# syzhang092218-source/dgppo

Measured on AMD Instinct MI355X. Metric: env-steps/sec whole node, LidarSpread n=8 4096 envs, 1/2/4/8 GPUs, higher is better.
Workload: dtype f32

## Files before the change

dgppo_amd/csrc/nn_dense.hip:

```cpp
#include "common.h"
#include "nn_gru.h"

using f32x4 = __attribute__((ext_vector_type(4))) float;
#ifdef DGPPO_STAMPS
__device__ unsigned long long g_dstamps[32];
#define DSTAMP(i) do { if (blockIdx.x == 0 && threadIdx.x == 0) g_dstamps[i] = __builtin_amdgcn_s_memtime(); } while (0)
extern "C" int32_t dgppo_debug_stamps_dense(unsigned long long* out) {
  return (int32_t)hipMemcpyFromSymbol(out, HIP_SYMBOL(g_dstamps), sizeof(unsigned long long) * 32);
}
#else
#define DSTAMP(i)
#endif

#define DENSE_ROWS 64

struct DenseArgs {
  const float* X; int ldx;
  const float* W; int ldw;
  const float* bias;
  float* Y; int ldy;
  int M, K, N;
  int act;
  int accumulate;
  int trans_w;
// ... 1015 lines not shown
  const float* dhn;
  float* dWi; int ldwi;
  float* dbi;
  float* dWh; int ldwh;
  float* dbhn;
  int M, rows_per_block;
  float* part;
  const float* dhs;
  const float* gates;
  float* dgi_out;
  GruH0Map hmap;
};

template <bool T1>
__global__ void __launch_bounds__(512) gru_bwd_w_kernel(GruBwdWArgs a) {
  extern __shared__ float sm[];
  const int tid = threadIdx.x, lane = tid & 63, wave = (tid >> 6) & 3, half = tid >> 8;
  const int li = lane & 15, lq = lane >> 4;
  const int m_begin = blockIdx.x * a.rows_per_block;
  const int m_end = min(a.M, m_begin + a.rows_per_block);
  f32x4 acc[12];
#pragma unroll
  for (int t = 0; t < 12; ++t) acc[t] = f32x4{0.f, 0.f, 0.f, 0.f};
  float4 pfa[2], pfy[T1 ? 6 : 4];
  float4 csum[T1 ? 4 : 1];
#pragma unroll
  for (int u = 0; u < (T1 ? 4 : 1); ++u) csum[u] = make_float4(0.f, 0.f, 0.f, 0.f);
  const int qa = tid & 31, ra = tid >> 5, qy = tid & 63, ry = tid >> 6;
  const int q1 = tid & 15, r1 = tid >> 4;
  auto hrow = [&](int row) -> const float* {
    if constexpr (T1) { if (a.hmap.n_inner.d > 0) return gru_h0_map_row(a.hprev, a.hmap, row); }
    return a.hprev + (size_t)row * a.ldh;
  };
  auto fetch = [&](int m0) {
#pragma unroll
    for (int u = 0; u < 2; ++u) {
      int row = m0 + u * 16 + ra;
      row = row < a.M ? row : a.M - 1;
      const float* src = qa < 16 ? a.x + (size_t)row * a.ldx + 4 * qa : hrow(row) + 4 * (qa - 16);
      pfa[u] = *reinterpret_cast<const float4*>(src);
    }
    if constexpr (T1) {
      int row = m0 + r1;
      row = row < a.M ? row : a.M - 1;
      pfy[0] = *reinterpret_cast<const float4*>(a.dhs + (size_t)row * 64 + 4 * q1);
      pfy[1] = *reinterpret_cast<const float4*>(hrow(row) + 4 * q1);
      const float* gs = a.gates + (size_t)row * 256 + 4 * q1;
#pragma unroll
      for (int g = 0; g < 4; ++g) pfy[2 + g] = *reinterpret_cast<const float4*>(gs + 64 * g);
    } else {
#pragma unroll
      for (int u = 0; u < 4; ++u) {
        int row = m0 + u * 8 + ry;
        row = row < a.M ? row : a.M - 1;
        const float* src = qy < 48 ? a.dgi + (size_t)row * 192 + 4 * qy : a.dhn + (size_t)row * 64 + 4 * (qy - 48);
        pfy[u] = *reinterpret_cast<const float4*>(src);
      }
    }
  };
  auto commit = [&](int m0, int b) {
    float* as = sm + b * GW_BUF;
    float* ys = as + BW_ROWS * GW_AL;
#pragma unroll
    for (int u = 0; u < 2; ++u) {
      const int r = u * 16 + ra;
      const float4 v = (m0 + r < m_end) ? pfa[u] : make_float4(0.f, 0.f, 0.f, 0.f);
      *reinterpret_cast<float4*>(as + r * GW_AL + 4 * qa) = v;
    }
    if constexpr (T1) {
      const bool in = m0 + r1 < m_end;
      const GruGateGrad g0 = gru_gate_grad(gru_zero_carry(pfy[0].x), pfy[1].x, pfy[2].x, pfy[3].x, pfy[4].x, pfy[5].x);
      const GruGateGrad g1 = gru_gate_grad(gru_zero_carry(pfy[0].y), pfy[1].y, pfy[2].y, pfy[3].y, pfy[4].y, pfy[5].y);
      const GruGateGrad g2 = gru_gate_grad(gru_zero_carry(pfy[0].z), pfy[1].z, pfy[2].z, pfy[3].z, pfy[4].z, pfy[5].z);
      const GruGateGrad g3 = gru_gate_grad(gru_zero_carry(pfy[0].w), pfy[1].w, pfy[2].w, pfy[3].w, pfy[4].w, pfy[5].w);
      float4 v[4] = {make_float4(g0.dar, g1.dar, g2.dar, g3.dar), make_float4(g0.daz, g1.daz, g2.daz, g3.daz),
                     make_float4(g0.dan, g1.dan, g2.dan, g3.dan), make_float4(g0.dhn, g1.dhn, g2.dhn, g3.dhn)};
      if (in) {
        float* o = a.dgi_out + (size_t)(m0 + r1) * 192 + 4 * q1;
#pragma unroll
        for (int g = 0; g < 3; ++g) *reinterpret_cast<float4*>(o + 64 * g) = v[g];
      }
#pragma unroll
      for (int g = 0; g < 4; ++g) {
        if (!in) v[g] = make_float4(0.f, 0.f, 0.f, 0.f);
        *reinterpret_cast<float4*>(ys + r1 * GW_YL + 64 * g + 4 * q1) = v[g];
        csum[g].x += v[g].x; csum[g].y += v[g].y; csum[g].z += v[g].z; csum[g].w += v[g].w;
      }
    } else {
#pragma unroll
      for (int u = 0; u < 4; ++u) {
        const int r = u * 8 + ry;
        const float4 v = (m0 + r < m_end) ? pfy[u] : make_float4(0.f, 0.f, 0.f, 0.f);
        *reinterpret_cast<float4*>(ys + r * GW_YL + 4 * qy) = v;
        csum[0].x += v.x; csum[0].y += v.y; csum[0].z += v.z; csum[0].w += v.w;
      }
    }
  };
  auto compute = [&](int b) {
    const float* as = sm + b * GW_BUF + lq * GW_AL + half * 64 + wave * 16 + li;
    const float* ys = sm + b * GW_BUF + BW_ROWS * GW_AL + lq * GW_YL + li;
    const float* yh = ys + (half ? 64 : 0);
#pragma unroll
    for (int s4 = 0; s4 < BW_ROWS / 4; ++s4) {
      float bv[12];
#pragma unroll
      for (int t = 0; t < 8; ++t) bv[t] = ys[s4 * 4 * GW_YL + t * 16];
#pragma unroll
      for (int t = 8; t < 12; ++t) bv[t] = yh[s4 * 4 * GW_YL + t * 16];
      const float av = as[s4 * 4 * GW_AL];
#pragma unroll
      for (int t = 0; t < 12; ++t) acc[t] = __builtin_amdgcn_mfma_f32_16x16x4f32(av, bv[t], acc[t], 0, 0, 0);
    }
  };
  fetch(m_begin);
  commit(m_begin, 0);
  __syncthreads();
  int cur = 0;
  for (int m0 = m_begin; m0 < m_end; m0 += BW_ROWS) {
    fetch(m0 + BW_ROWS);
    __builtin_amdgcn_sched_barrier(0);
    compute(cur);
    commit(m0 + BW_ROWS, cur ^ 1);
    asm volatile("s_waitcnt lgkmcnt(0)\n\ts_barrier" ::: "memory");
    cur ^= 1;
  }
  float* slab = a.part ? a.part + (size_t)blockIdx.x * GW_SLAB : nullptr;
  {
    float* out = half ? a.dWh : a.dWi;
    const int ldo = half ? a.ldwh : a.ldwi;
    float* sl = slab ? slab + (half ? GW_SLAB_WH : GW_SLAB_WI) : nullptr;
#pragma unroll
    for (int t = 0; t < 12; ++t) {
      const int col = t * 16 + li;
#pragma unroll
      for (int r = 0; r < 4; ++r) {
        const int krow = wave * 16 + lq * 4 + r;
// ... 193 lines not shown
```

dgppo_amd/csrc/nn_fused.hip:

```cpp
#include <type_traits>
#include "common.h"
#include "nn_ln.h"

using f32x4 = __attribute__((ext_vector_type(4))) float;
#define FZ_H 64
#define FZ_HL 66
#define FZ_RB 32
#define FZ_LDS_BARRIER() asm volatile("s_waitcnt lgkmcnt(0)\n\ts_barrier" ::: "memory")

__device__ inline float row16_sum(float v) {
  v += __int_as_float(__builtin_amdgcn_update_dpp(0, __float_as_int(v), 0xB1, 0xf, 0xf, false));
  v += __int_as_float(__builtin_amdgcn_update_dpp(0, __float_as_int(v), 0x4E, 0xf, 0xf, false));
  v += __int_as_float(__builtin_amdgcn_update_dpp(0, __float_as_int(v), 0x141, 0xf, 0xf, false));
  v += __int_as_float(__builtin_amdgcn_update_dpp(0, __float_as_int(v), 0x140, 0xf, 0xf, false));
  return v;
}

struct MlpGiArgs {
  const float* X; int ldx; int M;
  const float *W1, *b1, *g1, *be1, *W2, *b2, *g2, *be2, *Wi, *bi;
  float *p1, *y1, *st1, *p2, *y2, *st2;
  float* gi;
};

__global__ void __launch_bounds__(256) __attribute__((amdgpu_waves_per_eu(2, 8))) mlp_gi_fwd_kernel(MlpGiArgs a) {
// ... 1417 lines not shown
    else hipLaunchKernelGGL(gru1_head_fwd_rw_kernel<false>, dim3(grid_rw), dim3(64 * RW_WAVES), smem_rw, (hipStream_t)stream, a);
    DGPPO_LAUNCH_CHECK();
    return 0;
  }
  const size_t smem = sizeof(float) * 3 * FZ_RB * FZ_HL;
  const void* fn = two ? reinterpret_cast<const void*>(&gru1_head_fwd_kernel<true>)
                       : reinterpret_cast<const void*>(&gru1_head_fwd_kernel<false>);
  static thread_local int cap[2] = {0, 0};
  if (cap[two] == 0) {
    int per_cu = 0, dev = 0, cus = 256;
    if (hipOccupancyMaxActiveBlocksPerMultiprocessor(&per_cu, fn, 256, smem) != hipSuccess || per_cu < 1) per_cu = 1;
    if (hipGetDevice(&dev) != hipSuccess ||
        hipDeviceGetAttribute(&cus, hipDeviceAttributeMultiprocessorCount, dev) != hipSuccess || cus < 1) cus = 256;
    cap[two] = per_cu * cus;
  }
  const int tiles = (M + FZ_RB - 1) / FZ_RB;
  const int grid = tiles < cap[two] ? tiles : cap[two];
  if (two) hipLaunchKernelGGL(gru1_head_fwd_kernel<true>, dim3(grid), dim3(256), smem, (hipStream_t)stream, a);
  else hipLaunchKernelGGL(gru1_head_fwd_kernel<false>, dim3(grid), dim3(256), smem, (hipStream_t)stream, a);
  DGPPO_LAUNCH_CHECK();
  return 0;
}

#define HB_HL 68
#define HB_WAVES 8
#define HB_TILE (16 * HB_HL)
#define HB_BIG 1088
#define HB_SLAB_ONE HB_BIG
#define HB_SLAB_TWO (HB_BIG + FZ_H * FZ_H + FZ_H)
struct HeadBwdArgs {
  const float* feat; int ldf;
  const float* u;
  const float* dout; int n_out;
  const float *W1, *W2;
  float* dhs;
  float* dW1; int ldw1; float* db1;
  float* dW2; int ldw2; float* db2;
  float* part;
  int M;
};

template <bool TWO>
__global__ void __launch_bounds__(64 * HB_WAVES) head_bwd_kernel(HeadBwdArgs a) {
  extern __shared__ float sm[];
  const int tid = threadIdx.x, lane = tid & 63, w = tid >> 6, li = lane & 15, lq = lane >> 4;
  float* s_f = sm + w * 3 * HB_TILE;
// ... 244 lines not shown
```

dgppo_amd/engine.py:

```python
from __future__ import annotations

import dataclasses
from typing import Callable, Dict, Optional

import numpy as np
import os
import torch

from . import _native as N
from . import nets
from . import ops_algo as OA
from . import ops_env as OE
from . import ops_nn as K
from .utils import checkpoint as CK


@dataclasses.dataclass
class Hyper:
    gamma: float = 0.99
    gae_lambda: float = 0.95
    clip_eps: float = 0.25
    coef_ent: float = 1e-2
    max_grad_norm: float = 2.0
    lr_actor: float = 3e-4
# ... 404 lines not shown
                continue
            HC = self.HC
            hstar = self._final_carry(ro, e0, Eb)
            restore = False
            if not self.hp.use_rnn:
                h0 = None
            elif HC == H and self.carry_in_place:
                s0 = 0 if ro.stochastic else 1
                tm = ro._rnn_all
                if ro.stochastic:
                    tm[T + 1, e0:e0 + Eb].copy_(tm[T, e0:e0 + Eb])
                tm[s0 + T, e0:e0 + Eb].copy_(hstar.view(Eb, n, H))
                h0 = K.H0Map(tm[s0, e0:], tm.stride(1), tm.stride(0), T + 1, n, Eb, n_env_src=B - e0)
                restore = ro.stochastic
            elif HC == H:
                s0 = 0 if ro.stochastic else 1
                ro._rnn_em[e0:e0 + Eb, s0 + T].copy_(hstar.view(Eb, n, H))
                h0 = K.H0Blocks(ro._rnn_em[e0, s0], (T + 1) * n, (T + 2) * n * H, Eb)
            else:
                h0_all = self.arena.get("pre.h0all", Eb, T + 1, n, H)
                h0_all[:, :T].copy_(self._vh_carry(ro, e0, Eb))
                h0_all[:, T].copy_(hstar.view(Eb, n, HC)[..., :H])
                h0 = h0_all.view(-1, H)
            act = self.Vh.forward(feats, n_seq=Eb * (T + 1) * n, T=1, h0=h0, tag="pre", train=False)
            Vh_buf[e0:e0 + Eb].copy_(act["v"].view(Eb, T + 1, n, nh))
            if restore:
                ro._rnn_all[T, e0:e0 + Eb].copy_(ro._rnn_all[T + 1, e0:e0 + Eb])
        return Vl_buf, Vh_buf

    def require_landscape(self, what: str = "vh_landscape"):
        if self.algo != "dgppo":
            why = {"informarl_lagr": "its constraint-value net carries its own scan state, which needs a sequence pass first"}
            raise ValueError(f"{what}: algo '{self.algo}' is not supported: "
                             + why.get(self.algo, "it has no constraint-value network"))
        if self.cfg.is_vmas:
            raise ValueError(f"{what}: VMASReverseTransport is not supported")

    def vh_landscape(self, ro: RolloutData, env_index: int, agent_id: int, frame_ids, xs, ys,
                     events: Optional[list] = None) -> torch.Tensor:
        self.require_landscape()
        cfg, T = self.cfg, self.T
        n, nh, H = cfg.n_agents, self.n_cost, nets.HID
        ro.finalize()
        if not 0 <= int(env_index) < ro.B:
            raise ValueError(f"vh_landscape: env_index {env_index} outside [0, {ro.B})")
        if not 0 <= int(agent_id) < n:
            raise ValueError(f"vh_landscape: agent_id {agent_id} outside [0, {n})")
# ... 893 lines not shown
```

dgppo_amd/nets.py:

```python
from __future__ import annotations

import math
from typing import Dict, List, Optional, Tuple

import numpy as np
import torch

from . import _native as N
from . import ops_nn as K

H_HEADS = 3
MSG_DIM = 32
OUT_DIM = 64
HID = 64


def _ceil4(x):
    return (x + 3) // 4 * 4


class Layout:
    def __init__(self):
        self.entries: Dict[str, Tuple[int, Tuple[int, ...]]] = {}
        self.size = 0
# ... 192 lines not shown
    def pg(self, name):
        return self._cached("pg", self.prep_layout, self.prep_grads, name)

    def prepare(self):
        for l, (f, fp, d, kp) in enumerate(self.dims):
            q = lambda nm: self.p(f"gnn{l}.{nm}")
            K.gnn_prep(q("Wq"), q("bq"), q("Wk"), q("Wv"), q("bv"), q("We"), q("Wu"), self.pp(f"gnn{l}.Mcat"),
                       self.pp(f"gnn{l}.cvec"), self.pp(f"gnn{l}.Wout"), f, fp, d, H_HEADS, kp)

    def _xo_fusable(self, l: int) -> bool:
        if l != 0 or self.gnn_layers != 2:
            return False
        key = "_xo_ok"
        if not hasattr(self, key):
            f1, fp1, d1, kp1 = self.dims[1]
            setattr(self, key, self.dims[0][1] == 8 and self.dims[0][2] == 32 and fp1 == 32 and
                    K.attn_xo_supported(self.cfg, fp1, H_HEADS, kp1))
        return getattr(self, key)

    def zero_grads(self):
        self.grads.zero_()

    def forward(self, feats: GraphFeats, n_seq: int, T: int, h0: Optional[torch.Tensor], tag: str = "f",
                hs_out: Optional[torch.Tensor] = None, train: bool = True, qt0: Optional[torch.Tensor] = None):
        cfg, G, A = self.cfg, feats.G, self.arena
        n = cfg.n_agents
        R = G * n
        Ro = G * feats.n_other
        act = {"feats": feats, "G": G, "n_seq": n_seq, "T": T}
        Xa, Xo = feats.Xa, feats.Xo
        xo_fused = None
        for l, (f, fp, d, kp) in enumerate(self.dims):
            if l == 0 and qt0 is not None:
                assert tuple(qt0.shape) == (R, H_HEADS * fp), (tuple(qt0.shape), R, H_HEADS * fp)
                qt = qt0
            else:
                qt = A.get(f"{tag}.qt{l}", R, H_HEADS * fp)
                K.dense_fwd(Xa, self.pp(f"gnn{l}.Mcat"), self.pp(f"gnn{l}.cvec"), qt)
            zcat = A.get(f"{tag}.zcat{l}", R, kp)
            lean = l == 0 and self.lean_attn0 and feats.edges_from_rows
            attn = A.get(f"{tag}.attn{l}", R, cfg.fan_in, H_HEADS) if train and not lean else None
            if lean:
                K.attn_fwd_rows(cfg, fp, H_HEADS, kp, qt, Xa, Xo if Ro > 0 else None, feats.emask, zcat, None, G)
            elif xo_fused is not None:
                K.attn_fwd_xo(cfg, fp, H_HEADS, kp, qt, Xa, xo_fused[0], xo_fused[1], xo_fused[2], feats.efeat, feats.emask, zcat, attn, G)
            else:
                K.attn_fwd(cfg, fp, H_HEADS, kp, qt, Xa, Xo if Ro > 0 else None, feats.efeat, feats.emask, zcat, attn, G)
# ... 41 lines not shown
            saves = None
            if train:
                saves = tuple(A.get(f"{tag}.{nm}{i}", Rh, w) for i in (1, 2) for nm, w in (("p", HID), ("y", HID), ("st", 2)))
                for i in (1, 2):
                    act[f"p{i}"], act[f"y{i}"], act[f"st{i}"] = saves[3 * (i - 1):3 * i]
            K.mlp_gi_fwd(x, self.p("mlp.W1"), self.p("mlp.b1"), self.p("mlp.g1"), self.p("mlp.be1"), self.p("mlp.W2"),
                         self.p("mlp.b2"), self.p("mlp.g2"), self.p("mlp.be2"), self.p("gru.Wi"), self.p("gru.bi"), gi, saves)
        assert n_seq * T == Rh, (n_seq, T, Rh)
        L, CD = self.rnn_layers, self.carry_dim
        h0_blocks = isinstance(h0, K.H0Blocks)
        if h0_blocks:
            assert self.rnn == "gru" and L == 1 and T == 1 and not train and self.kind != "policy", \
                "a blocked h0 serves the one-cell GRU value nets' T = 1 inference pass"
        h0_map = isinstance(h0, K.H0Map)
        if h0_map:
            assert self.rnn == "gru" and L == 1 and T == 1 and self.kind != "policy" and h0.n_inner == n_inner, \
                "a mapped h0 serves the one-cell GRU value nets' T = 1 passes"
        elif h0 is not None and not h0_blocks:
            assert tuple(h0.shape) == (n_seq, CD), (tuple(h0.shape), n_seq, CD)
        if hs_out is not None:
            assert tuple(hs_out.shape) == (Rh, CD), (tuple(hs_out.shape), Rh, CD)
        act["gi"] = gi
        simple = (self.rnn == "gru" and L == 1)
        if simple:
            hs = hs_out if hs_out is not None else A.get(f"{tag}.hs", Rh, HID)
            hprev_is_h0 = train and T == 1 and h0 is not None and self.kind != "policy"
            hprev = A.get(f"{tag}.hprev", Rh, HID) if (train and not hprev_is_h0) else None
            gates = A.get(f"{tag}.gates", Rh, 4 * HID) if train else None
            feat = hs
            act["hs"], act["hprev"], act["gates"] = hs, hprev, gates
        fused_tail = (simple and T == 1 and self.kind == "policy")
        if simple and not fused_tail:
            if h0_blocks:
                K.gru_fwd_h0_blocks(gi, self.p("gru.Wh"), self.p("gru.bhn"), h0, hs, hprev, gates, n_seq, T, n_inner)
            elif h0_map:
                K.gru_fwd_h0_map(gi, self.p("gru.Wh"), self.p("gru.bhn"), h0, hs, hprev, gates, n_seq, T, n_inner)
            else:
                K.gru_fwd(gi, self.p("gru.Wh"), self.p("gru.bhn"), h0, hs, hprev, gates, n_seq, T, n_inner)
            if hprev_is_h0:
                act["hprev"] = act["h0"] = h0
        if self.rnn == "none":
            feat = act["y2"]
            if hs_out is not None:
                if h0 is not None and T == 1:
                    hs_out.copy_(h0)
                else:
                    hs_out.zero_()
        elif self.rnn == "lstm":
            x_l = act["y2"]
            act["stack"] = []
            for l in range(L):
                zi = A.get(f"{tag}.zi{l}", Rh, 4 * HID)
                for half in (slice(0, 2 * HID), slice(2 * HID, 4 * HID)):
                    K.dense_fwd(x_l, self.p(f"lstm{l}.Wi")[:, half], None, zi[:, half])
                c0_l = h0_l = None
# ... 25 lines not shown
                if h0 is not None:
                    h0_l = A.get(f"{tag}.h0_{l}", n_seq, HID)
                    h0_l.copy_(h0[:, l * HID:(l + 1) * HID])
                hs_l = A.get(f"{tag}.hs{l}", Rh, HID)
                hprev_l = A.get(f"{tag}.hprev{l}", Rh, HID) if train else None
                gates_l = A.get(f"{tag}.gates{l}", Rh, 4 * HID) if train else None
                K.gru_fwd(gi_l, self.p(f"{pre}.Wh"), self.p(f"{pre}.bhn"), h0_l, hs_l, hprev_l, gates_l, n_seq, T, n_inner)
                if hs_out is not None:
                    hs_out[:, l * HID:(l + 1) * HID].copy_(hs_l)
                act["stack"].append(dict(x=x_l, gi=gi_l, hs=hs_l, hprev=hprev_l, gates=gates_l))
                x_l = hs_l
            feat = x_l
        act["feat"] = feat
        if self.kind == "policy":
            u = A.get(f"{tag}.u", Rh, HID) if (train or not fused_tail) else None
            ms = A.get(f"{tag}.ms", Rh, 4)
            if fused_tail:
                K.gru1_head_fwd(gi, self.p("gru.Wh"), self.p("gru.bhn"), h0, self.p("head.Ws"), self.p("head.bs"),
                                self.p("head.Wms"), self.p("head.bms"), hs, hprev, gates, u, ms)
            else:
                K.dense_fwd(feat, self.p("head.Ws"), self.p("head.bs"), u)
                K.dense_fwd(u, self.p("head.Wms"), self.p("head.bms"), ms)
            act["u"], act["ms"] = u, ms
        else:
            v = A.get(f"{tag}.v", Rh, self.n_out)
            K.dense_fwd(feat, self.p("head.Wo"), self.p("head.bo"), v)
            act["v"] = v
        return act

    def backward(self, act, dout: torch.Tensor, tag: str = "b"):
        A = self.arena
        ws_floats = getattr(self, "_bwdw_floats", 16 << 20)

        def _alloc(n_floats):
            self._bwdw_floats = max(ws_floats, n_floats)
            return self.ws_arena.get(f"{tag}.bwdw_ws", self._bwdw_floats)
        batch = K.BwdWBatch(self.device, _alloc) if dout.is_cuda else None
        if batch is not None:
            batch.__enter__()
        try:
            self._backward_body(act, dout, tag)
        except BaseException:
            if batch is not None:
                batch.__exit__(RuntimeError, None, None)
            raise
        if batch is not None:
            batch.__exit__(None, None, None)
# ... 243 lines not shown
```

dgppo_amd/ops_nn.py:

```python
from __future__ import annotations

import ctypes as C
from typing import Optional

import numpy as np
import torch

from . import _native as N

FLOPS = [0.0]


def _mat(t: torch.Tensor, name: str):
    if t.dim() != 2:
        raise ValueError(f"{name} must be 2-D, got {tuple(t.shape)}")
    if not t.is_cuda:
        raise RuntimeError(f"{name} must live on the GPU (the HIP path has no CPU fallback)")
    if t.dtype != torch.float32:
        raise TypeError(f"{name} must be float32")
    if t.shape[1] > 1 and t.stride(1) != 1:
        raise ValueError(f"{name} must have unit inner stride")
    ld = t.stride(0) if t.shape[0] > 1 else max(t.shape[1], t.stride(0))
    return C.c_void_p(t.data_ptr()), int(ld), int(t.shape[0]), int(t.shape[1])

# ... 827 lines not shown
        flat = torch.as_strided(self.base, (self.base.untyped_storage().nbytes() // 4 - self.base.storage_offset(),), (1,))
        return flat[(off[:, None] + torch.arange(64, device=dev)[None, :])].contiguous()

    def _args(self):
        return (C.c_void_p(self.base.data_ptr()), C.c_void_p(self.ids.data_ptr()) if self.ids is not None else None,
                self.n_env, self.n_time)


def gru_fwd_h0_map(gi, Wh, bhn, h0: H0Map, hs, hprev, gates, n_seq, T, n_inner):
    if T != 1 or n_inner != h0.n_inner:
        raise ValueError(f"a mapped h0 serves one-step passes of its own n_inner = {h0.n_inner} (got T = {T}, n_inner = {n_inner})")
    N.expect_shape(gi, (n_seq, 192), "gi")
    N.expect_shape(hs, (n_seq, 64), "hs")
    N.expect_shape(Wh, (64, 192), "Wh")
    if n_seq > h0.n_seq:
        raise ValueError(f"h0: the map holds {h0.n_seq} carries, fewer than n_seq = {n_seq}")
    FLOPS[0] += 2.0 * n_seq * 64 * 192
    base, ids, n_env, n_time = h0._args()
    rc = N.lib().dgppo_gru_fwd_h0_map(_p(gi), _p(Wh), _p(bhn), base, ids, n_env, n_time, C.c_int64(h0.env_stride),
                                      C.c_int64(h0.time_stride), _p(hs), _p(hprev), _p(gates), n_seq, n_inner, N.stream_ptr())
    N.check(rc, "dgppo_gru_fwd_h0_map")


class GatherDesc(C.Structure):
    _fields_ = [("src", C.c_void_p), ("dst", C.c_void_p), ("row_bytes", C.c_int64), ("src_stride", C.c_int64)]


GATHER_MAX = 8


def gather_rows(pairs, ids):
    if ids.dtype != torch.int32 or not ids.is_cuda or not ids.is_contiguous():
        raise TypeError("ids must be a contiguous int32 CUDA tensor")
    n_ids = int(ids.numel())
    if len(pairs) > GATHER_MAX:
        raise ValueError(f"gather_rows takes at most {GATHER_MAX} tensors per launch, got {len(pairs)}")
    descs = (GatherDesc * max(len(pairs), 1))()
    for k, (src, dst) in enumerate(pairs):
        if not (src.is_cuda and dst.is_cuda):
            raise RuntimeError("gather_rows: tensors must live on the GPU (the HIP path has no CPU fallback)")
        if src.dtype != dst.dtype or tuple(dst.shape) != (n_ids,) + tuple(src.shape[1:]):
            raise ValueError(f"gather_rows: pair {k}: dst {tuple(dst.shape)} {dst.dtype} does not fit src {tuple(src.shape)} "
                             f"{src.dtype} gathered by {n_ids} ids")
        if not dst.is_contiguous() or (src.shape[0] > 0 and not src[0].is_contiguous()):
            raise ValueError(f"gather_rows: pair {k}: dst and the rows of src must be contiguous")
        row = (src[0].numel() if src.shape[0] > 0 else 0) * src.element_size()
# ... 231 lines not shown
```

include/dgppo_hip.h:

```cpp
#ifndef DGPPO_HIP_H
#define DGPPO_HIP_H

#include <stdint.h>

#ifdef __cplusplus
extern "C" {
#endif

#define DGPPO_ABI_VERSION 3

enum {
  DGPPO_ENV_LIDAR_SPREAD = 0,
  DGPPO_ENV_LIDAR_TARGET = 1,
  DGPPO_ENV_LIDAR_BICYCLE_TARGET = 2,
  DGPPO_ENV_MPE_SPREAD = 3,
  DGPPO_ENV_MPE_TARGET = 4,
  DGPPO_ENV_LIDAR_LINE = 5,
  DGPPO_ENV_MPE_LINE = 6,
  DGPPO_ENV_MPE_FORMATION = 7,
  DGPPO_ENV_MPE_CORRIDOR = 8,
  DGPPO_ENV_MPE_CONNECT_SPREAD = 9,
  DGPPO_ENV_VMAS_REVERSE_TRANSPORT = 10
};
enum {
// ... 273 lines not shown
                             int32_t ldwo, const float* bo, const float* efeat, float* dqt, float* dXa, float* dWo,
                             int32_t lddwo, float* dbo, float* workspace, int64_t workspace_bytes, int32_t G, void* stream);

int32_t dgppo_gnn_prep(const float* Wq, const float* bq, const float* Wk, const float* Wv, const float* bv,
                       const float* We, const float* Wu, float* Mcat, float* cvec, float* Wout, int32_t F, int32_t Fp,
                       int32_t D, int32_t H, int32_t Kp, void* stream);
int32_t dgppo_gnn_unprep(const float* dMcat, const float* dcvec, const float* dWout, const float* Wq, const float* bq,
                         const float* Wk, float* dWq, float* dbq, float* dWk, float* dWv, float* dbv, float* dWe,
                         float* dWu, int32_t F, int32_t Fp, int32_t D, int32_t H, int32_t Kp, void* stream);

int32_t dgppo_ln_relu_fwd(const float* x, const float* gamma, const float* beta, float* y, float* stats, int32_t M,
                          void* stream);
int32_t dgppo_ln_relu_bwd(const float* x, const float* y, const float* stats, const float* gamma, const float* dy,
                          float* dx, float* dgamma, float* dbeta, int32_t M, void* stream);

int32_t dgppo_gru_fwd(const float* gi, const float* Wh, const float* bhn, const float* h0, float* hs, float* hprev,
                      float* gates, int32_t n_seq, int32_t T, int32_t n_inner, void* stream);
int32_t dgppo_gru_fwd_h0_blocks(const float* gi, const float* Wh, const float* bhn, const float* h0,
                                int32_t rows_per_block, int64_t block_stride, float* hs, float* hprev, float* gates,
                                int32_t n_seq, int32_t T, int32_t n_inner, void* stream);
int32_t dgppo_gru_fwd_h0_map(const float* gi, const float* Wh, const float* bhn, const float* h0, const int32_t* ids,
                             int32_t n_env, int32_t n_time, int64_t env_stride, int64_t time_stride, float* hs,
                             float* hprev, float* gates, int32_t n_seq, int32_t n_inner, void* stream);
int32_t dgppo_gru_bwd(const float* dhs, const float* Wh, const float* hprev, const float* gates, float* dgi,
                      float* dgh, int32_t n_seq, int32_t T, int32_t n_inner, void* stream);
int32_t dgppo_gru_bwd_dhn(const float* dhs, const float* Wh, const float* hprev, const float* gates, float* dgi,
                          float* dhn, int32_t n_seq, int32_t T, int32_t n_inner, void* stream);
int64_t dgppo_gru_bwd_w_workspace_bytes(void);
int32_t dgppo_gru_bwd_w(const float* x, int32_t ldx, const float* hprev, int32_t ldh, const float* dgi, const float* dhn,
                        float* dWi, int32_t ldwi, float* dbi, float* dWh, int32_t ldwh, float* dbhn, int32_t M,
                        float* workspace, int64_t workspace_bytes, dgppo_reduce_desc* pending, void* stream);
int32_t dgppo_gru_bwd_w_t1(const float* x, int32_t ldx, const float* h0, int32_t ldh, const float* dhs, const float* gates,
                           float* dgi, float* dWi, int32_t ldwi, float* dbi, float* dWh, int32_t ldwh, float* dbhn, int32_t M,
                           float* workspace, int64_t workspace_bytes, dgppo_reduce_desc* pending, void* stream);
int32_t dgppo_gru_bwd_w_t1_map(const float* x, int32_t ldx, const float* h0, const int32_t* ids, int32_t n_env, int32_t n_time,
                               int32_t n_inner, int64_t env_stride, int64_t time_stride, const float* dhs, const float* gates,
                               float* dgi, float* dWi, int32_t ldwi, float* dbi, float* dWh, int32_t ldwh, float* dbhn,
                               int32_t M, float* workspace, int64_t workspace_bytes, dgppo_reduce_desc* pending, void* stream);

int32_t dgppo_lstm_fwd(const float* zi, const float* Wh, const float* bh, const float* c0, const float* h0, float* cs,
                       float* hs, float* cprev, float* hprev, float* gates, int32_t n_seq, int32_t T, int32_t n_inner,
                       void* stream);
int32_t dgppo_lstm_bwd(const float* dhs, const float* Wh, const float* cprev, const float* gates, float* dz,
                       int32_t n_seq, int32_t T, int32_t n_inner, void* stream);

int32_t dgppo_policy_head(const float* ms, const float* eps, const float* action_in, float* action, float* log_pi,
// ... 43 lines not shown
```

Before: 4.984 million.

## Fuse single-step GRU with value head Dense and drop unused hidden-state output

Adds a kernel that runs a one-step GRU together with the value-head Dense projection in a single launch. It stages Wh and Wo in LDS, prefetches the next tile's gi and h0, and can skip writing hs when the caller does not need it. The value-net pre-pass now uses this path with need_hs=False. The T1 backward-weights kernel also reuses the h0 row already loaded for the gate gradient instead of reloading it, and precomputes the mapped env id one tile ahead. This removes a kernel launch and a round trip of hs through memory, at the cost of more code paths, falling back to the old route for misaligned operands or mid-range M.

```diff
diff --git a/dgppo_amd/csrc/nn_dense.hip b/dgppo_amd/csrc/nn_dense.hip
--- a/dgppo_amd/csrc/nn_dense.hip
+++ b/dgppo_amd/csrc/nn_dense.hip
@@ -1061,14 +1061,28 @@
   f32x4 acc[12];
 #pragma unroll
   for (int t = 0; t < 12; ++t) acc[t] = f32x4{0.f, 0.f, 0.f, 0.f};
-  float4 pfa[2], pfy[T1 ? 6 : 4];
+  float4 pfa[2] = {make_float4(0.f, 0.f, 0.f, 0.f), make_float4(0.f, 0.f, 0.f, 0.f)}, pfy[T1 ? 6 : 4];
   float4 csum[T1 ? 4 : 1];
 #pragma unroll
   for (int u = 0; u < (T1 ? 4 : 1); ++u) csum[u] = make_float4(0.f, 0.f, 0.f, 0.f);
   const int qa = tid & 31, ra = tid >> 5, qy = tid & 63, ry = tid >> 6;
   const int q1 = tid & 15, r1 = tid >> 4;
+  const bool mapped_ids = T1 && a.hmap.n_inner.d > 0 && a.hmap.ids != nullptr;
+  int idn = 0;
+  auto id_of = [&](int m0) -> int {
+    int row = m0 + r1;
+    row = row < a.M ? row : a.M - 1;
+    return a.hmap.ids[gru_div(gru_div((unsigned)row, a.hmap.n_inner), a.hmap.n_time)];
+  };
   auto hrow = [&](int row) -> const float* {
-    if constexpr (T1) { if (a.hmap.n_inner.d > 0) return gru_h0_map_row(a.hprev, a.hmap, row); }
+    if constexpr (T1) {
+      if (a.hmap.n_inner.d > 0) {
+        if (!mapped_ids) return gru_h0_map_row(a.hprev, a.hmap, row);
+        const unsigned c = gru_div((unsigned)row, a.hmap.n_inner), ag = (unsigned)row - c * (unsigned)a.hmap.n_inner.d;
+        const unsigned t = c - gru_div(c, a.hmap.n_time) * (unsigned)a.hmap.n_time.d;
+        return a.hprev + (long)idn * a.hmap.env_stride + (long)t * a.hmap.time_stride + (long)ag * 64;
+      }
+    }
     return a.hprev + (size_t)row * a.ldh;
   };
   auto fetch = [&](int m0) {
@@ -1076,14 +1090,19 @@
     for (int u = 0; u < 2; ++u) {
       int row = m0 + u * 16 + ra;
       row = row < a.M ? row : a.M - 1;
-      const float* src = qa < 16 ? a.x + (size_t)row * a.ldx + 4 * qa : hrow(row) + 4 * (qa - 16);
-      pfa[u] = *reinterpret_cast<const float4*>(src);
+      if constexpr (T1) {
+        if (qa < 16) pfa[u] = *reinterpret_cast<const float4*>(a.x + (size_t)row * a.ldx + 4 * qa);
+      } else {
+        const float* src = qa < 16 ? a.x + (size_t)row * a.ldx + 4 * qa : hrow(row) + 4 * (qa - 16);
+        pfa[u] = *reinterpret_cast<const float4*>(src);
+      }
     }
     if constexpr (T1) {
       int row = m0 + r1;
       row = row < a.M ? row : a.M - 1;
       pfy[0] = *reinterpret_cast<const float4*>(a.dhs + (size_t)row * 64 + 4 * q1);
       pfy[1] = *reinterpret_cast<const float4*>(hrow(row) + 4 * q1);
+      if (mapped_ids) idn = id_of(m0 + BW_ROWS);
       const float* gs = a.gates + (size_t)row * 256 + 4 * q1;
 #pragma unroll
       for (int g = 0; g < 4; ++g) pfy[2 + g] = *reinterpret_cast<const float4*>(gs + 64 * g);
@@ -1104,10 +1123,11 @@
     for (int u = 0; u < 2; ++u) {
       const int r = u * 16 + ra;
       const float4 v = (m0 + r < m_end) ? pfa[u] : make_float4(0.f, 0.f, 0.f, 0.f);
-      *reinterpret_cast<float4*>(as + r * GW_AL + 4 * qa) = v;
+      if (!T1 || qa < 16) *reinterpret_cast<float4*>(as + r * GW_AL + 4 * qa) = v;
     }
     if constexpr (T1) {
       const bool in = m0 + r1 < m_end;
+      *reinterpret_cast<float4*>(as + r1 * GW_AL + 64 + 4 * q1) = in ? pfy[1] : make_float4(0.f, 0.f, 0.f, 0.f);
       const GruGateGrad g0 = gru_gate_grad(gru_zero_carry(pfy[0].x), pfy[1].x, pfy[2].x, pfy[3].x, pfy[4].x, pfy[5].x);
       const GruGateGrad g1 = gru_gate_grad(gru_zero_carry(pfy[0].y), pfy[1].y, pfy[2].y, pfy[3].y, pfy[4].y, pfy[5].y);
       const GruGateGrad g2 = gru_gate_grad(gru_zero_carry(pfy[0].z), pfy[1].z, pfy[2].z, pfy[3].z, pfy[4].z, pfy[5].z);
@@ -1151,6 +1171,7 @@
       for (int t = 0; t < 12; ++t) acc[t] = __builtin_amdgcn_mfma_f32_16x16x4f32(av, bv[t], acc[t], 0, 0, 0);
     }
   };
+  if (mapped_ids) idn = id_of(m_begin);
   fetch(m_begin);
   commit(m_begin, 0);
   __syncthreads();
diff --git a/dgppo_amd/csrc/nn_fused.hip b/dgppo_amd/csrc/nn_fused.hip
--- a/dgppo_amd/csrc/nn_fused.hip
+++ b/dgppo_amd/csrc/nn_fused.hip
@@ -1,6 +1,7 @@
 #include <type_traits>
 #include "common.h"
 #include "nn_ln.h"
+#include "nn_gru.h"
 
 using f32x4 = __attribute__((ext_vector_type(4))) float;
 #define FZ_H 64
@@ -1464,6 +1465,252 @@
   return 0;
 }
 
+struct GruStepArgs {
+  const float *gi, *Wh, *bhn, *h0;
+  const float *Wo, *bo;
+  float *hs, *hprev, *gates, *out;
+  int M, n_out;
+  GruFastDiv rpb; long bstride;
+  GruH0Map map; int n_env;
+};
+
+struct GruStepGate { float rg, zg, ng, hn, hnew; };
+__device__ __forceinline__ GruStepGate gru_step_gate(float gr, float gz, float gn, float ar, float az, float an, float bn, float hp) {
+#pragma clang fp contract(off)
+  GruStepGate o;
+  o.rg = gate_sigmoid(gr + ar);
+  o.zg = gate_sigmoid(gz + az);
+  o.hn = an + bn;
+  o.ng = gate_tanh(__fmaf_rn(o.rg, o.hn, gn));
+  o.hnew = __fmaf_rn(o.zg, hp, (1.0f - o.zg) * o.ng);
+  return o;
+}
+
+__device__ __forceinline__ int gru_step_env(const GruStepArgs& a, int s) {
+  const unsigned c = gru_div((unsigned)s, a.map.n_inner), e = gru_div(c, a.map.n_time);
+  return (int)e < a.n_env ? (int)e : a.n_env - 1;
+}
+__device__ __forceinline__ const float* gru_step_h0_row(const GruStepArgs& a, int s, long env) {
+  if (a.map.n_inner.d > 0) {
+    const unsigned c = gru_div((unsigned)s, a.map.n_inner), ag = (unsigned)s - c * (unsigned)a.map.n_inner.d;
+    const unsigned e = gru_div(c, a.map.n_time), t = c - e * (unsigned)a.map.n_time.d;
+    return a.h0 + env * a.map.env_stride + (long)t * a.map.time_stride + (long)ag * 64;
+  }
+  if (a.rpb.d > 0) {
+    const unsigned b = gru_div((unsigned)s, a.rpb);
+    return a.h0 + (long)b * a.bstride + (long)((unsigned)s - b * (unsigned)a.rpb.d) * 64;
+  }
+  return a.h0 + (size_t)s * 64;
+}
+
+#define GSH_WOL 17
+#define GSH_PAIR_M0 131072
+#define GSH_PAIR_M1 1048576
+#define GSH_YL_SAVE 100
+#define GSH_SMEM_FLOATS(yl) (64 * RW_WIL + 64 * GSH_WOL + 80 + RW_WAVES * 16 * (yl))
+template <bool SAVE>
+__global__ void __launch_bounds__(64 * RW_WAVES) gru_step_head_kernel(GruStepArgs a) {
+  extern __shared__ float sm[];
+  constexpr int YL = SAVE ? GSH_YL_SAVE : RW_YL;
+  float* sWh = sm;
+  float* sWo = sWh + 64 * RW_WIL;
+  float* sB = sWo + 64 * GSH_WOL;
+  const int tid = threadIdx.x, lane = tid & 63, w = tid >> 6, li = lane & 15, lq = lane >> 4;
+  float* sY = sB + 80 + w * (16 * YL);
+  const int n_tiles = (a.M + 15) >> 4, stride = gridDim.x * RW_WAVES;
+  const bool has_h0 = a.h0 != nullptr, ids = a.map.n_inner.d > 0 && a.map.ids != nullptr;
+  int tile = w * gridDim.x + blockIdx.x;
+  auto srow = [&](int t) { return t < n_tiles ? min(t * 16 + li, a.M - 1) : a.M - 1; };
+  auto env_of = [&](int s) -> long {
+    return a.map.n_inner.d > 0 ? (long)gru_step_env(a, s) : 0L;
+  };
+  float H[16], G[4][4][3];
+  auto fetch_h0 = [&](const float* p) {
+    const float4* q = reinterpret_cast<const float4*>(p + lq * 16);
+#pragma unroll
+    for (int j = 0; j < 4; ++j) { const float4 v = q[j]; H[4 * j] = v.x; H[4 * j + 1] = v.y; H[4 * j + 2] = v.z; H[4 * j + 3] = v.w; }
+  };
+  auto fetch_gi = [&](int t) {
+#pragma unroll
+    for (int r = 0; r < 4; ++r) {
+      const int row = min(t * 16 + lq * 4 + r, a.M - 1);
+      const float* gp = a.gi + (size_t)row * 192 + li;
+#pragma unroll
+      for (int ct = 0; ct < 4; ++ct) { G[ct][r][0] = gp[ct * 16]; G[ct][r][1] = gp[64 + ct * 16]; G[ct][r][2] = gp[128 + ct * 16]; }
+    }
+  };
+#pragma unroll
+  for (int j = 0; j < 16; ++j) H[j] = 0.0f;
+  int idn = 0;
+  if (tile < n_tiles) {
+    if (has_h0) {
+      const int s = srow(tile);
+      long env = env_of(s);
+      if (ids) { env = a.map.ids[env]; idn = a.map.ids[gru_step_env(a, srow(tile + stride))]; }
+      fetch_h0(gru_step_h0_row(a, s, env));
+    }
+    fetch_gi(tile);
+  }
+  {
+    static_assert(RW_WAVES == 16, "the staging below assumes 1024 threads");
+    float4 vh[3];
+#pragma unroll
+    for (int j = 0; j < 3; ++j) vh[j] = reinterpret_cast<const float4*>(a.Wh)[j * 1024 + tid];
+    const int k = tid >> 4, c = tid & 15;
+    const float wo = (c < a.n_out) ? a.Wo[k * a.n_out + c] : 0.0f;
+#pragma unroll
+    for (int j = 0; j < 3; ++j) {
+      const int q = j * 1024 + tid, kq = q / 48, cq = (q - kq * 48) * 4;
+      float* d = sWh + kq * RW_WIL + cq;
+      d[0] = vh[j].x; d[1] = vh[j].y; d[2] = vh[j].z; d[3] = vh[j].w;
+    }
+    sWo[k * GSH_WOL + c] = wo;
+    if (tid < 64) sB[tid] = a.bhn[tid];
+    if (tid < 16) sB[64 + tid] = (tid < a.n_out) ? a.bo[tid] : 0.0f;
+  }
+  __syncthreads();
+  for (; tile < n_tiles; tile += stride) {
+    const int row0 = tile * 16, nxt = tile + stride;
+    const bool more = nxt < n_tiles;
+    const float* pn = a.h0;
+#pragma unroll
+    for (int j = 0; j < 4; ++j)
+      *reinterpret_cast<float4*>(sY + li * YL + lq * 16 + 4 * j) = make_float4(H[4 * j], H[4 * j + 1], H[4 * j + 2], H[4 * j + 3]);
+    if (SAVE && a.hprev != nullptr && row0 + li < a.M) {
+      float4* hp4 = reinterpret_cast<float4*>(a.hprev + (size_t)(row0 + li) * 64 + lq * 16);
+#pragma unroll
+      for (int j = 0; j < 4; ++j) hp4[j] = make_float4(H[4 * j], H[4 * j + 1], H[4 * j + 2], H[4 * j + 3]);
+    }
+    asm volatile("" ::: "memory");
+#pragma unroll
+    for (int ct = 0; ct < 4; ++ct) {
+      f32x4 ar = f32x4{0.f, 0.f, 0.f, 0.f}, az = ar, an = ar;
+#pragma unroll
+      for (int kk = 0; kk < 16; ++kk) {
+        const float* wr = sWh + (lq * 16 + kk) * RW_WIL + ct * 16 + li;
+        ar = __builtin_amdgcn_mfma_f32_16x16x4f32(H[kk], wr[0], ar, 0, 0, 0);
+        az = __builtin_amdgcn_mfma_f32_16x16x4f32(H[kk], wr[64], az, 0, 0, 0);
+        an = __builtin_amdgcn_mfma_f32_16x16x4f32(H[kk], wr[128], an, 0, 0, 0);
+      }
+      const float bn = sB[ct * 16 + li];
+      float gk[2][4];
+#pragma unroll
+      for (int r = 0; r < 4; ++r) {
+        float* e = sY + (lq * 4 + r) * YL + ct * 16 + li;
+        const GruStepGate g = gru_step_gate(G[ct][r][0], G[ct][r][1], G[ct][r][2], ar[r], az[r], an[r], bn, *e);
+        *e = g.hnew;
+        if (SAVE) { e[64 - ct * 16] = g.rg; e[80 - ct * 16] = g.zg; }
+        gk[0][r] = g.ng; gk[1][r] = g.hn;
+      }
+      if (SAVE && a.gates != nullptr) {
+#pragma unroll
+        for (int half = 0; half < 2; ++half) {
+          if (half == 1) {
+#pragma unroll
+            for (int r = 0; r < 4; ++r) {
+              float* d = sY + (lq * 4 + r) * YL + 64 + li;
+              d[0] = gk[0][r]; d[16] = gk[1][r];
+            }
+          }
+          asm volatile("" ::: "memory");
+          const float4 v0 = *reinterpret_cast<const float4*>(sY + li * YL + 64 + lq * 8);
+          const float4 v1 = *reinterpret_cast<const float4*>(sY + li * YL + 64 + lq * 8 + 4);
+          if (row0 + li < a.M) {
+            float4* gp = reinterpret_cast<float4*>(a.gates + (size_t)(row0 + li) * 256 + (2 * half + (lq >> 1)) * 64 + ct * 16 + (lq & 1) * 8);
+            gp[0] = v0; gp[1] = v1;
+          }
+          asm volatile("" ::: "memory");
+        }
+      }
+      if (ct == 1 && more && has_h0) {
+        const int s = srow(nxt);
+        pn = gru_step_h0_row(a, s, ids ? (long)idn : env_of(s));
+        if (ids) idn = a.map.ids[gru_step_env(a, srow(nxt + stride))];
+      }
+    }
+    if (more) {
+      fetch_gi(nxt);
+      if (has_h0) fetch_h0(pn);
+    }
+    float A[16];
+    asm volatile("" ::: "memory");
+#pragma unroll
+    for (int j = 0; j < 4; ++j) {
+      const float4 v = *reinterpret_cast<const float4*>(sY + li * YL + lq * 16 + 4 * j);
+      A[4 * j] = v.x; A[4 * j + 1] = v.y; A[4 * j + 2] = v.z; A[4 * j + 3] = v.w;
+    }
+    asm volatile("" ::: "memory");
+    if (a.hs != nullptr && row0 + li < a.M) {
+      float4* h4 = reinterpret_cast<float4*>(a.hs + (size_t)(row0 + li) * 64 + lq * 16);
+#pragma unroll
+      for (int j = 0; j < 4; ++j) h4[j] = make_float4(A[4 * j], A[4 * j + 1], A[4 * j + 2], A[4 * j + 3]);
+    }
+    f32x4 ao = f32x4{0.f, 0.f, 0.f, 0.f};
+#pragma unroll
+    for (int kk = 0; kk < 16; ++kk) ao = __builtin_amdgcn_mfma_f32_16x16x4f32(A[kk], sWo[(lq * 16 + kk) * GSH_WOL + li], ao, 0, 0, 0);
+    const float b = sB[64 + li];
+#pragma unroll
+    for (int r = 0; r < 4; ++r) {
+      const int row = row0 + lq * 4 + r;
+      if (row < a.M && li < a.n_out) a.out[(size_t)row * a.n_out + li] = ao[r] + b;
+    }
+  }
+}
+
+extern "C" int32_t dgppo_gru_step_head_fwd(const float* gi, const float* Wh, const float* bhn, const float* h0,
+                                           int32_t rows_per_block, int64_t block_stride, const int32_t* ids, int32_t n_env,
+                                           int32_t n_time, int32_t n_inner, int64_t env_stride, int64_t time_stride,
+                                           const float* Wo, const float* bo, float* hs, float* hprev, float* gates, float* out,
+                                           int32_t M, int32_t n_out, void* stream) {
+  DGPPO_REQUIRE(M >= 0 && n_out >= 1 && n_out <= 16, "gru_step_head_fwd: bad shape M=%d n_out=%d", M, n_out);
+  DGPPO_REQUIRE(gi && Wh && bhn && Wo && bo && out, "gru_step_head_fwd: NULL operand");
+  const bool mapped = n_time > 0, blocked = !mapped && rows_per_block > 0;
+  DGPPO_REQUIRE(!(mapped && rows_per_block > 0), "gru_step_head_fwd: h0 is either blocked or mapped");
+  DGPPO_REQUIRE(mapped || ids == nullptr, "gru_step_head_fwd: ids without a map");
+  if (mapped || blocked) DGPPO_REQUIRE(h0 != nullptr && ((uintptr_t)h0 & 15) == 0, "gru_step_head_fwd: a blocked or mapped h0 must be a 16-byte aligned pointer");
+  if (blocked)
+    DGPPO_REQUIRE(block_stride >= (int64_t)rows_per_block * 64 && block_stride % 4 == 0,
+                  "gru_step_head_fwd: block_stride must be a multiple of 4 and >= rows_per_block * 64");
+  if (mapped) {
+    DGPPO_REQUIRE(n_env >= 1 && n_inner >= 1, "gru_step_head_fwd: bad sizes n_env=%d n_time=%d n_inner=%d", n_env, n_time, n_inner);
+    DGPPO_REQUIRE(env_stride % 4 == 0 && time_stride % 4 == 0 && env_stride >= 0 && time_stride >= 0,
+                  "gru_step_head_fwd: env_stride and time_stride must be non-negative multiples of 4 floats");
+    DGPPO_REQUIRE((int64_t)M <= (int64_t)n_env * n_time * n_inner, "gru_step_head_fwd: the map holds fewer than M = %d carries", M);
+  }
+  if (M == 0) return 0;
+  const uintptr_t al = reinterpret_cast<uintptr_t>(gi) | reinterpret_cast<uintptr_t>(Wh) | reinterpret_cast<uintptr_t>(h0) |
+                       reinterpret_cast<uintptr_t>(hs) | reinterpret_cast<uintptr_t>(hprev) | reinterpret_cast<uintptr_t>(gates);
+  if ((al & 15) != 0 || (M >= GSH_PAIR_M0 && M < GSH_PAIR_M1)) {
+    DGPPO_REQUIRE(hs != nullptr, "gru_step_head_fwd: the scan kernel and the head Dense (operands off a 16-byte boundary, or 131072 <= M < 1048576) need hs");
+    int32_t rc;
+    if (mapped) rc = dgppo_gru_fwd_h0_map(gi, Wh, bhn, h0, ids, n_env, n_time, env_stride, time_stride, hs, hprev, gates, M, n_inner, stream);
+    else if (blocked) rc = dgppo_gru_fwd_h0_blocks(gi, Wh, bhn, h0, rows_per_block, block_stride, hs, hprev, gates, M, 1, 1, stream);
+    else rc = dgppo_gru_fwd(gi, Wh, bhn, h0, hs, hprev, gates, M, 1, 1, stream);
+    if (rc) return rc;
+    return dgppo_dense_fwd(hs, 64, Wo, n_out, bo, out, n_out, M, 64, n_out, 0, 0, 0, nullptr, 0, stream);
+  }
+  GruStepArgs a{};
+  a.gi = gi; a.Wh = Wh; a.bhn = bhn; a.h0 = h0; a.Wo = Wo; a.bo = bo;
+  a.hs = hs; a.hprev = hprev; a.gates = gates; a.out = out; a.M = M; a.n_out = n_out;
+  if (blocked) { a.rpb = gru_fast_div(rows_per_block); a.bstride = (long)block_stride; }
+  if (mapped) { a.map = gru_h0_map(ids, (long)env_stride, (long)time_stride, n_inner, n_time); a.n_env = n_env; }
+  const bool save = hprev != nullptr || gates != nullptr;
+  const size_t smem = sizeof(float) * (save ? GSH_SMEM_FLOATS(GSH_YL_SAVE) : GSH_SMEM_FLOATS(RW_YL));
+  static thread_local bool attr[2] = {false, false};
+  if (!attr[save]) {
+    const void* f = save ? reinterpret_cast<const void*>(&gru_step_head_kernel<true>)
+                         : reinterpret_cast<const void*>(&gru_step_head_kernel<false>);
+    const hipError_t e = hipFuncSetAttribute(f, hipFuncAttributeMaxDynamicSharedMemorySize, (int)smem);
+    DGPPO_REQUIRE(e == hipSuccess, "gru_step_head_fwd: cannot reserve %zu bytes of LDS per workgroup: %s", smem, hipGetErrorString(e));
+    attr[save] = true;
+  }
+  const int cus = head_bwd_cus(), tiles16 = (M + 15) / 16, grid = tiles16 < cus ? tiles16 : cus;
+  if (save) hipLaunchKernelGGL(gru_step_head_kernel<true>, dim3(grid), dim3(64 * RW_WAVES), smem, (hipStream_t)stream, a);
+  else hipLaunchKernelGGL(gru_step_head_kernel<false>, dim3(grid), dim3(64 * RW_WAVES), smem, (hipStream_t)stream, a);
+  DGPPO_LAUNCH_CHECK();
+  return 0;
+}
+
 #define HB_HL 68
 #define HB_WAVES 8
 #define HB_TILE (16 * HB_HL)
diff --git a/dgppo_amd/engine.py b/dgppo_amd/engine.py
--- a/dgppo_amd/engine.py
+++ b/dgppo_amd/engine.py
@@ -450,7 +450,7 @@
                 h0_all[:, :T].copy_(self._vh_carry(ro, e0, Eb))
                 h0_all[:, T].copy_(hstar.view(Eb, n, HC)[..., :H])
                 h0 = h0_all.view(-1, H)
-            act = self.Vh.forward(feats, n_seq=Eb * (T + 1) * n, T=1, h0=h0, tag="pre", train=False)
+            act = self.Vh.forward(feats, n_seq=Eb * (T + 1) * n, T=1, h0=h0, tag="pre", train=False, need_hs=False)
             Vh_buf[e0:e0 + Eb].copy_(act["v"].view(Eb, T + 1, n, nh))
             if restore:
                 ro._rnn_all[T, e0:e0 + Eb].copy_(ro._rnn_all[T + 1, e0:e0 + Eb])
diff --git a/dgppo_amd/nets.py b/dgppo_amd/nets.py
--- a/dgppo_amd/nets.py
+++ b/dgppo_amd/nets.py
@@ -238,7 +238,8 @@
         self.grads.zero_()
 
     def forward(self, feats: GraphFeats, n_seq: int, T: int, h0: Optional[torch.Tensor], tag: str = "f",
-                hs_out: Optional[torch.Tensor] = None, train: bool = True, qt0: Optional[torch.Tensor] = None):
+                hs_out: Optional[torch.Tensor] = None, train: bool = True, qt0: Optional[torch.Tensor] = None,
+                need_hs: bool = True):
         cfg, G, A = self.cfg, feats.G, self.arena
         n = cfg.n_agents
         R = G * n
@@ -326,15 +327,25 @@
             assert tuple(hs_out.shape) == (Rh, CD), (tuple(hs_out.shape), Rh, CD)
         act["gi"] = gi
         simple = (self.rnn == "gru" and L == 1)
+        step_head = (simple and T == 1 and self.kind != "policy")
         if simple:
-            hs = hs_out if hs_out is not None else A.get(f"{tag}.hs", Rh, HID)
+            drop_hs = (step_head and not need_hs and hs_out is None and not train
+                       and K.gru_step_head_rw(gi, self.p("gru.Wh"), h0, None, None, None))
+            hs = hs_out if hs_out is not None else (None if drop_hs else A.get(f"{tag}.hs", Rh, HID))
             hprev_is_h0 = train and T == 1 and h0 is not None and self.kind != "policy"
             hprev = A.get(f"{tag}.hprev", Rh, HID) if (train and not hprev_is_h0) else None
             gates = A.get(f"{tag}.gates", Rh, 4 * HID) if train else None
             feat = hs
             act["hs"], act["hprev"], act["gates"] = hs, hprev, gates
         fused_tail = (simple and T == 1 and self.kind == "policy")
-        if simple and not fused_tail:
+        if step_head:
+            v = A.get(f"{tag}.v", Rh, self.n_out)
+            K.gru_step_head_fwd(gi, self.p("gru.Wh"), self.p("gru.bhn"), h0, self.p("head.Wo"), self.p("head.bo"), hs, hprev,
+                                gates, v)
+            act["v"] = v
+            if hprev_is_h0:
+                act["hprev"] = act["h0"] = h0
+        elif simple and not fused_tail:
             if h0_blocks:
                 K.gru_fwd_h0_blocks(gi, self.p("gru.Wh"), self.p("gru.bhn"), h0, hs, hprev, gates, n_seq, T, n_inner)
             elif h0_map:
@@ -406,7 +417,7 @@
                 K.dense_fwd(feat, self.p("head.Ws"), self.p("head.bs"), u)
                 K.dense_fwd(u, self.p("head.Wms"), self.p("head.bms"), ms)
             act["u"], act["ms"] = u, ms
-        else:
+        elif not step_head:
             v = A.get(f"{tag}.v", Rh, self.n_out)
             K.dense_fwd(feat, self.p("head.Wo"), self.p("head.bo"), v)
             act["v"] = v
diff --git a/dgppo_amd/ops_nn.py b/dgppo_amd/ops_nn.py
--- a/dgppo_amd/ops_nn.py
+++ b/dgppo_amd/ops_nn.py
@@ -873,6 +873,50 @@
     N.check(rc, "dgppo_gru_fwd_h0_map")
 
 
+def _h0_ptr(h0) -> int:
+    if h0 is None:
+        return 0
+    return (h0.base if isinstance(h0, (H0Blocks, H0Map)) else h0).data_ptr()
+
+
+def gru_step_head_rw(gi, Wh, h0, hs, hprev, gates) -> bool:
+    ptrs = [gi.data_ptr(), Wh.data_ptr(), _h0_ptr(h0)] + [t.data_ptr() for t in (hs, hprev, gates) if t is not None]
+    M = gi.shape[0]
+    return all(p % 16 == 0 for p in ptrs) and not 131072 <= M < 1048576
+
+
+def gru_step_head_fwd(gi, Wh, bhn, h0, Wo, bo, hs, hprev, gates, out):
+    M, n_out = gi.shape[0], out.shape[1]
+    N.expect_shape(gi, (M, 192), "gi"); N.expect_shape(Wh, (64, 192), "Wh"); N.expect_shape(bhn, (64,), "bhn")
+    N.expect_shape(Wo, (64, n_out), "Wo"); N.expect_shape(bo, (n_out,), "bo"); N.expect_shape(out, (M, n_out), "out")
+    if not 1 <= n_out <= 16:
+        raise ValueError(f"gru_step_head_fwd: n_out must be in [1, 16], got {n_out}")
+    for t, shp, nm in ((hs, (M, 64), "hs"), (hprev, (M, 64), "hprev"), (gates, (M, 256), "gates")):
+        if t is not None:
+            N.expect_shape(t, shp, nm)
+    rpb, bstride, ids, n_env, n_time, n_inner, es, ts = 0, 0, None, 0, 0, 0, 0, 0
+    if isinstance(h0, H0Blocks):
+        if M > h0.n_seq:
+            raise ValueError(f"h0: {h0.n_blocks} blocks of {h0.rows_per_block} rows hold fewer than M = {M} carries")
+        hp, rpb, bstride = C.c_void_p(h0.base.data_ptr()), h0.rows_per_block, h0.block_stride
+    elif isinstance(h0, H0Map):
+        if M > h0.n_seq:
+            raise ValueError(f"h0: the map holds {h0.n_seq} carries, fewer than M = {M}")
+        hp, ids, n_env, n_time = h0._args()
+        n_inner, es, ts = h0.n_inner, h0.env_stride, h0.time_stride
+    else:
+        if h0 is not None:
+            N.expect_shape(h0, (M, 64), "h0")
+        hp = _p(h0, "h0")
+    if hs is None and not gru_step_head_rw(gi, Wh, h0, hs, hprev, gates):
+        raise ValueError("gru_step_head_fwd: this call runs the scan kernel and the head Dense (alignment or M), which need hs")
+    FLOPS[0] += 2.0 * M * (64 * 192 + 64 * n_out)
+    rc = N.lib().dgppo_gru_step_head_fwd(_p(gi), _p(Wh), _p(bhn), hp, rpb, C.c_int64(bstride), ids, n_env, n_time, n_inner,
+                                         C.c_int64(es), C.c_int64(ts), _p(Wo), _p(bo), _p(hs), _p(hprev), _p(gates), _p(out),
+                                         M, n_out, N.stream_ptr())
+    N.check(rc, "dgppo_gru_step_head_fwd")
+
+
 class GatherDesc(C.Structure):
     _fields_ = [("src", C.c_void_p), ("dst", C.c_void_p), ("row_bytes", C.c_int64), ("src_stride", C.c_int64)]
 
diff --git a/include/dgppo_hip.h b/include/dgppo_hip.h
--- a/include/dgppo_hip.h
+++ b/include/dgppo_hip.h
@@ -319,6 +319,10 @@
 int32_t dgppo_gru_fwd_h0_map(const float* gi, const float* Wh, const float* bhn, const float* h0, const int32_t* ids,
                              int32_t n_env, int32_t n_time, int64_t env_stride, int64_t time_stride, float* hs,
                              float* hprev, float* gates, int32_t n_seq, int32_t n_inner, void* stream);
+int32_t dgppo_gru_step_head_fwd(const float* gi, const float* Wh, const float* bhn, const float* h0, int32_t rows_per_block,
+                                int64_t block_stride, const int32_t* ids, int32_t n_env, int32_t n_time, int32_t n_inner,
+                                int64_t env_stride, int64_t time_stride, const float* Wo, const float* bo, float* hs,
+                                float* hprev, float* gates, float* out, int32_t M, int32_t n_out, void* stream);
 int32_t dgppo_gru_bwd(const float* dhs, const float* Wh, const float* hprev, const float* gates, float* dgi,
                       float* dgh, int32_t n_seq, int32_t T, int32_t n_inner, void* stream);
 int32_t dgppo_gru_bwd_dhn(const float* dhs, const float* Wh, const float* hprev, const float* gates, float* dgi,
```

Result: no change. 5.027 million (median of 6 runs) (+0.8%).
